# patrickltobing/shallow-wavenet

Hardware: AMD Instinct MI355X
Metric: decoded samples/sec (22.05 kHz Laplacian AR decode, whole job) (higher is better)
Workload: dtype f32

## Files before the change

### shallow_wavenet_amd/csrc/swn_decode_bl6_common.hpp

```cpp
#pragma once
#include <hip/hip_runtime.h>
#include "swn_decode_internal.hpp"

namespace swn_bl6 {

constexpr int NT = 512;
constexpr int H = 64;
constexpr int L = 6;
constexpr int RF = 64;
#ifdef SWN_STAMP
constexpr bool HEADS_ON = false;
#else
constexpr bool HEADS_ON = true;
#endif

struct Bl6Args {
    const float* P;
    SwnLayout y;
    const float* cond;
    const float* noise;
    const void* forced;
    void* out;
    float* heads;
    int B, Tf, n_steps, U, N;
    SwnNoise nz;
    const void* seed;
    int step0, resume;
    float* sess;
};

struct Bl6PoolArgs {
    Bl6Args c;
    SwnPoolTable t;
};
static_assert(sizeof(Bl6PoolArgs) <= 4096, "kernel arguments are limited to 4 KB");
struct Bl6PoolModelsArgs : Bl6PoolArgs {
    SwnPoolModels m;
};
static_assert(sizeof(Bl6PoolModelsArgs) <= 4096, "kernel arguments are limited to 4 KB");
struct Bl6W16Args : Bl6Args {
    const void* w16;
};
struct Bl6PoolW16Args : Bl6PoolArgs {
    const void* w16;
};
static_assert(sizeof(Bl6PoolW16Args) <= 4096, "kernel arguments are limited to 4 KB");
struct Bl6W16Layout {
    size_t wsk, w1, w2, total;
};
inline __host__ __device__ Bl6W16Layout w16_layout(int S, int O1, int NO, bool softmax) {
    Bl6W16Layout y;
    y.wsk = 0;
    y.w1 = y.wsk + (size_t)L * S * 64 * 2;
    y.w2 = y.w1 + (size_t)O1 * S * 2;
    y.total = y.w2 + (softmax ? (size_t)NO * O1 * 2 : 0);
    return y;
}

constexpr int cmax(int a, int b) { return a > b ? a : b; }
constexpr int pow2ceil(int x) { int r = 1; while (r < x) r <<= 1; return r; }
constexpr int r4(int x) { return (x + 3) & ~3; }

__device__ __forceinline__ __amdgpu_buffer_rsrc_t make_rsrc(const void* p, unsigned bytes) {
    return __builtin_amdgcn_make_buffer_rsrc(const_cast<void*>(p), 0, bytes, 0x00020000);
}
__device__ __forceinline__ float4 buf_ld4(__amdgpu_buffer_rsrc_t r, unsigned voff_bytes, unsigned soff_bytes) {
    return __builtin_bit_cast(float4, __builtin_amdgcn_raw_buffer_load_b128(r, voff_bytes, soff_bytes, 0));
}
__device__ __forceinline__ uint4 buf_ld4u(__amdgpu_buffer_rsrc_t r, unsigned voff_bytes, unsigned soff_bytes) {
    return __builtin_bit_cast(uint4, __builtin_amdgcn_raw_buffer_load_b128(r, voff_bytes, soff_bytes, 0));
}
__device__ __forceinline__ float w16_lo(unsigned w) { return __builtin_bit_cast(float, w << 16); }
__device__ __forceinline__ float w16_hi(unsigned w) { return __builtin_bit_cast(float, w & 0xffff0000u); }

template <int CTRL>
__device__ __forceinline__ float dpp_f(float v) {
    return __builtin_bit_cast(float, __builtin_amdgcn_update_dpp(0, __builtin_bit_cast(int, v), CTRL, 0xf, 0xf, true));
}
__device__ __forceinline__ float sum4(float v) {
    v += dpp_f<0xB1>(v);
    v += dpp_f<0x4E>(v);
    return v;
}
__device__ __forceinline__ float sum8(float v) {
    v = sum4(v);
    v += dpp_f<0x141>(v);
    return v;
}
__device__ __forceinline__ float exp_c(float x) {
    const float t = x * 1.44269504f;
    const float lo = fmaf(x, 1.44269504f, -t) + x * 1.92596299e-8f;
    const float e = __builtin_amdgcn_exp2f(t);
    return fmaf(e, lo * 0.693147181f, e);
}
__device__ __forceinline__ float rcp_c(float x) {
    const float r = __builtin_amdgcn_rcpf(x);
    return fmaf(r, fmaf(-x, r, 1.f), r);
}
__device__ __forceinline__ float sigm(float x) { return rcp_c(1.f + exp_c(-x)); }
__device__ __forceinline__ float tanh_c(float x) {
    if (fabsf(x) > 9.02f) return copysignf(1.f, x);
    const float t = exp_c(-2.f * fabsf(x));
    return copysignf((1.f - t) * rcp_c(1.f + t), x);
}
__device__ __forceinline__ float ssign(float x) { return x * rcp_c(1.f + fabsf(x)); }

__device__ __forceinline__ void lds_barrier() {
#ifdef SWN_SYNC
    __syncthreads(); return;
#endif
    __builtin_amdgcn_fence(__ATOMIC_RELEASE, "workgroup", "local");
    __builtin_amdgcn_s_barrier();
    __builtin_amdgcn_fence(__ATOMIC_ACQUIRE, "workgroup", "local");
}

#define c_b  lds[T::o_cz + o]
#define c_v0 lds[T::o_cz + H + o]
#define c_v1 lds[T::o_cz + 2 * H + o]
#define c_c0 lds[T::o_cz + 3 * H + o]
#define c_c1 lds[T::o_cz + 4 * H + o]

inline void fill_args(Bl6Args& a, const SwnDecodeCall& c) {
    swn_make_layout(&c.g, &a.y);
    a.P = c.packed; a.cond = c.cond; a.noise = c.nz.ptr; a.nz = c.nz; a.forced = c.forced; a.seed = c.seed; a.out = c.out;
    a.heads = c.heads; a.B = c.batch; a.Tf = c.n_frames; a.n_steps = c.n_steps; a.U = c.g.U; a.N = c.g.N;
    a.step0 = c.step0; a.resume = c.resume; a.sess = c.stream ? c.state : nullptr;
}

inline bool wants_ext(const Bl6Args& a) { return !a.nz.ptr || a.nz.dump || a.seed; }

template <class A>
int launch_kernel(void (*kern)(A), size_t lds_bytes, int n_groups, const A& a, hipStream_t st, const char* where) {
    if (lds_bytes > 64 * 1024 &&
        hipFuncSetAttribute(reinterpret_cast<const void*>(kern), hipFuncAttributeMaxDynamicSharedMemorySize, (int)lds_bytes) != hipSuccess)
        return SWN_E_LAUNCH;
    hipLaunchKernelGGL(kern, dim3(n_groups), dim3(NT), lds_bytes, st, a);
    return swn_launch_status(where);
}

}
```

### shallow_wavenet_amd/csrc/swn_decode_bl6w.hip

```cpp
#include <type_traits>
#include "swn_decode_bl6_common.hpp"
#include "swn_decode_internal.hpp"

namespace {

using namespace swn_bl6;

constexpr int NG = 256;
constexpr int S = 128;
constexpr int O1 = 128;

template <int LPC_, bool EXT_>
struct Tw {
    static constexpr int LPC = LPC_;
    static constexpr bool EXT = EXT_;
    using Ext = Tw<LPC_, true>;
    static constexpr int NO = 2 + LPC_;
    static constexpr int WN = cmax(1, LPC_) + 1;
    static constexpr int ring_len(int l) { return pow2ceil((1 << l) + 1); }
    static constexpr int ring_off(int l) { int o = 0; for (int i = 0; i < l; ++i) o += ring_len(i) * H; return o; }
    static constexpr int PF = L * 2 * H;
    static constexpr int NZC = 64, NZB = 4;
    static constexpr int o_ring = 0;
    static constexpr int o_hcat = o_ring + ring_off(L);
    static constexpr int o_gp = o_hcat + L * H;
    static constexpr int o_bx = o_gp + 2 * PF;
    static constexpr int o_bd = o_bx + L * 2 * H;
    static constexpr int o_old = o_bd + L * 2 * H;
    static constexpr int o_wup = o_old + 2 * L * 2 * H;
    static constexpr int o_skip = o_wup + 256;
    static constexpr int o_p2 = o_skip + S;
    static constexpr int o_tnz = o_p2 + 4 * NO;
    static constexpr int o_cz = o_tnz + r4(NZB * NZC);
    static constexpr int o_w2 = o_cz + 5 * H;
    static constexpr int o_bias = o_w2 + NO * S + r4(NO);
    static constexpr int o_w1 = o_bias + S + O1;
    static constexpr int o_wl = o_w1 + 8 * O1 * 16;
    static constexpr int o_h0w = o_wl + 8 * NG * 4;
    static constexpr int o_end = o_h0w + 3 * H;
    static constexpr size_t lds_bytes = (size_t)o_end * sizeof(float);
    static constexpr int sess_old = ring_off(L);
    static constexpr int sess_win = sess_old + 2 * L * 2 * H;
    static constexpr int sess_floats = sess_win + r4(WN);
};

__device__ __forceinline__ float sum_quads(float v) {
    v += dpp_f<0x124>(v);
    v += dpp_f<0x128>(v);
    float w = v;
    asm("s_nop 1\n\tv_permlane16_swap_b32 %0, %1" : "+v"(v), "+v"(w));
    v += w;
    w = v;
    asm("s_nop 1\n\tv_permlane32_swap_b32 %0, %1" : "+v"(v), "+v"(w));
    return v + w;
}
template <class T, int LAYER>
__device__ __forceinline__ void layer_a(float* lds, const float (&w)[2][16], const int q, const float wj, const int pb, const int ta,
                                        const float* xr) {
    const int o = ta >> 2, p = ta & 3, pr = p & 1;
    const float e_old = lds[T::o_old + (q & 1) * (L * 2 * H) + LAYER * 2 * H + pr * H + o];
    const float e_gx = fmaf(wj, lds[T::o_gp + pb + LAYER * 2 * H + pr * H + o], lds[T::o_bx + LAYER * 2 * H + pr * H + o]);
    const float e_hp = xr[o];
    float az = 0.f, ac = 0.f;
#pragma unroll
    for (int m = 0; m < 4; ++m) {
        const float4 x = *reinterpret_cast<const float4*>(xr + 16 * p + 4 * m);
        az = fmaf(w[0][4 * m], x.x, az); ac = fmaf(w[1][4 * m], x.x, ac);
        az = fmaf(w[0][4 * m + 1], x.y, az); ac = fmaf(w[1][4 * m + 1], x.y, ac);
        az = fmaf(w[0][4 * m + 2], x.z, az); ac = fmaf(w[1][4 * m + 2], x.z, ac);
        az = fmaf(w[0][4 * m + 3], x.w, az); ac = fmaf(w[1][4 * m + 3], x.w, ac);
    }
    az = sum4(az); ac = sum4(ac);
    __builtin_amdgcn_sched_barrier(0);
    if (p < 2) {
        const float sa = (p == 0 ? az : ac) + e_old;
        const float v = e_gx * sa;
        float res;
        if (fabsf(v) > 9.02f && p == 1) {
            res = copysignf(1.f, v);
        } else {
            const float e = exp_c(p == 0 ? -v : -2.f * fabsf(v));
            const float r = rcp_c(1.f + e);
            res = p == 0 ? r : copysignf((1.f - e) * r, v);
        }
        const float c = dpp_f<0xF5>(res);
        if (p == 0) {
            const float hn = (1.f - res) * c + res * e_hp;
            if (LAYER + 1 < L) {
                constexpr int R2 = T::ring_len(LAYER + 1 < L ? LAYER + 1 : LAYER);
                lds[T::o_ring + T::ring_off(LAYER + 1 < L ? LAYER + 1 : LAYER) + (q & (R2 - 1)) * H + o] = hn;
            }
            lds[T::o_hcat + LAYER * H + o] = hn;
        }
    }
    __builtin_amdgcn_sched_barrier(0);
}

template <class T, int LAYER, int MB = 4>
__device__ __forceinline__ void older_sum(const float* lds, const float (&w)[2][16], const int qn, const int tb, float& az, float& ac) {
    constexpr int dil = 1 << LAYER;
    constexpr int R = T::ring_len(LAYER);
    const int p = tb & 3;
    const float* ring = lds + T::o_ring + T::ring_off(LAYER);
    az = 0.f; ac = 0.f;
#pragma unroll
    for (int m = 0; m < 4; ++m) {
        const float4 x = *reinterpret_cast<const float4*>(ring + ((qn - dil) & (R - 1)) * H + 16 * p + 4 * m);
        float4 w0, w1;
        if (LAYER < L - 1) {
            w0 = make_float4(w[0][4 * m], w[0][4 * m + 1], w[0][4 * m + 2], w[0][4 * m + 3]);
            w1 = make_float4(w[1][4 * m], w[1][4 * m + 1], w[1][4 * m + 2], w[1][4 * m + 3]);
        } else {
            w0 = *reinterpret_cast<const float4*>(lds + T::o_wl + (m * NG + tb) * 4);
            w1 = *reinterpret_cast<const float4*>(lds + T::o_wl + ((4 + m) * NG + tb) * 4);
        }
        az = fmaf(w0.x, x.x, az); ac = fmaf(w1.x, x.x, ac);
        az = fmaf(w0.y, x.y, az); ac = fmaf(w1.y, x.y, ac);
        az = fmaf(w0.z, x.z, az); ac = fmaf(w1.z, x.z, ac);
        az = fmaf(w0.w, x.w, az); ac = fmaf(w1.w, x.w, ac);
        if (MB < 4 && m % MB == MB - 1) __builtin_amdgcn_sched_barrier(0);
    }
    az = sum4(az); ac = sum4(ac);
}
template <class T, int LAYER>
__device__ __forceinline__ void older_store(float* lds, const int qn, const int tb, const float az, const float ac) {
    const int o = tb >> 2, p = tb & 3, pr = p & 1;
    lds[T::o_old + (qn & 1) * (L * 2 * H) + LAYER * 2 * H + pr * H + o] = (p == 0 ? az : ac) + lds[T::o_bd + LAYER * 2 * H + pr * H + o];
}
template <class T, int LAYER, int MB = 4>
__device__ __forceinline__ void older_b(float* lds, const float (&w)[2][16], const int qn, const int tb) {
    float az, ac;
    older_sum<T, LAYER, MB>(lds, w, qn, tb, az, ac);
    if ((tb & 3) < 2) older_store<T, LAYER>(lds, qn, tb, az, ac);
}
template <int... LS> struct Layers {};
template <class T, int NW, int... LS>
__device__ __forceinline__ void older_bn(Layers<LS...>, float* lds, const float (&w)[NW][2][16], const int qn, const int tb) {
    static_assert(((LS < NW) && ...), "register-resident halves only");
    float az[sizeof...(LS)], ac[sizeof...(LS)];
    int k = 0;
    ((older_sum<T, LS>(lds, w[LS], qn, tb, az[k], ac[k]), ++k), ...);
    if ((tb & 3) < 2) {
        k = 0;
        ((older_store<T, LS>(lds, qn, tb, az[k], ac[k]), ++k), ...);
    }
}

template <int LAYER>
__device__ __forceinline__ void skip_issue_b(__amdgpu_buffer_rsrc_t wsk2, float4 (&wsl)[8], const int tb, const unsigned step0) {
    const int r = tb >> 2, hp = tb & 3;
#pragma unroll
    for (int ps = 0; ps < 2; ++ps)
#pragma unroll
        for (int mm = 0; mm < 4; ++mm)
            wsl[ps * 4 + mm] = buf_ld4(wsk2, (unsigned)((r + 64 * ps) * 4 + hp) * 16u, (unsigned)((LAYER * 4 + mm) * S) * 64u + step0);
}
template <class T, int LAYER>
__device__ __forceinline__ void skip_roll_b(const float* lds, __amdgpu_buffer_rsrc_t wsk2, float4 (&wsl)[8], float (&sacc)[2], const int tb,
                                            const unsigned step0) {
    static_assert(LAYER >= 1 && LAYER < L, "slice LAYER - 1 in flight, slice LAYER to request");
    const int r = tb >> 2, hp = tb & 3;
#pragma unroll
    for (int hf = 0; hf < 2; ++hf) {
#pragma unroll
        for (int mm = 2 * hf; mm < 2 * hf + 2; ++mm) {
            const float4 x = *reinterpret_cast<const float4*>(lds + T::o_hcat + (LAYER - 1) * H + 16 * mm + 4 * hp);
#pragma unroll
            for (int ps = 0; ps < 2; ++ps) {
                const float4 w = wsl[ps * 4 + mm];
                sacc[ps] = fmaf(w.x, x.x, sacc[ps]); sacc[ps] = fmaf(w.y, x.y, sacc[ps]);
                sacc[ps] = fmaf(w.z, x.z, sacc[ps]); sacc[ps] = fmaf(w.w, x.w, sacc[ps]);
            }
        }
        __builtin_amdgcn_sched_barrier(0);
#pragma unroll
        for (int mm = 2 * hf; mm < 2 * hf + 2; ++mm)
#pragma unroll
            for (int ps = 0; ps < 2; ++ps)
                wsl[ps * 4 + mm] = buf_ld4(wsk2, (unsigned)((r + 64 * ps) * 4 + hp) * 16u, (unsigned)((LAYER * 4 + mm) * S) * 64u + step0);
        __builtin_amdgcn_sched_barrier(0);
    }
    asm volatile("" : "+v"(sacc[0]), "+v"(sacc[1]));
}
template <class T>
__device__ __forceinline__ void skip_last_b(float* lds, const float4 (&wsl)[8], const float (&sacc)[2], const int tb) {
    const int r = tb >> 2, hp = tb & 3;
    float part[2][4];
#pragma unroll
    for (int mm = 0; mm < 4; ++mm) {
        const float4 x = *reinterpret_cast<const float4*>(lds + T::o_hcat + (L - 1) * H + 16 * mm + 4 * hp);
#pragma unroll
        for (int ps = 0; ps < 2; ++ps) {
            const float4 w = wsl[ps * 4 + mm];
            part[ps][mm] = fmaf(w.w, x.w, fmaf(w.z, x.z, fmaf(w.y, x.y, w.x * x.x)));
        }
    }
    float s[2];
#pragma unroll
    for (int ps = 0; ps < 2; ++ps) s[ps] = sacc[ps] + ((part[ps][0] + part[ps][1]) + (part[ps][2] + part[ps][3]));
    const float t0 = s[0] + dpp_f<0xB1>(s[0]), t1 = s[1] + dpp_f<0xB1>(s[1]);
    const float v = (hp < 2 ? t0 : t1) + dpp_f<0x4E>(hp < 2 ? t1 : t0);
    if ((hp & 1) == 0) lds[T::o_skip + r + 32 * hp] = fmaxf(v, 0.f);
}

using OlderMerged = Layers<3, 4>;
using OlderOut1 = Layers<0, 1, 2>;

template <class T, bool GA, bool STREAM, bool POOL = false>
__device__ __forceinline__ void decode_body(const Bl6Args& a, float* lds) {
    constexpr bool EXT = T::EXT;
    static_assert(!STREAM || EXT, "streamed chunks run the extended mode");
    constexpr bool grpA = GA;
    const int tid = threadIdx.x, b = POOL ? 0 : blockIdx.x;
    __builtin_assume(GA ? tid < NG : tid >= NG);
    const int tg = tid & (NG - 1);
    const float* __restrict__ P = a.P;
    const int U = a.U;
    const int s0 = STREAM ? a.step0 : 0;
    const bool resume = STREAM && a.resume;
    const int fb0 = STREAM ? s0 / U : 0;

    for (int e = tid; e < T::o_end; e += NT) lds[e] = 0.f;
    __syncthreads();
    for (int e = tid; e < L * 2 * H; e += NT) {
        lds[T::o_bx + e] = P[a.y.bx + e];
        const float bd = P[a.y.bd + e];
        lds[T::o_bd + e] = bd;
        lds[T::o_old + e] = bd;
    }
    for (int e = tid; e < U; e += NT) lds[T::o_wup + e] = P[a.y.wup + e];
    for (int e = tid; e < H; e += NT) lds[T::o_cz + e] = P[a.y.cb + e];
    for (int e = tid; e < S; e += NT) lds[T::o_bias + e] = P[a.y.bsk + e];
    for (int e = tid; e < O1; e += NT) lds[T::o_bias + S + e] = P[a.y.b1 + e];
    for (int e = tid; e < 2 * H; e += NT) { lds[T::o_cz + H + e] = P[a.y.cv + e]; lds[T::o_cz + 3 * H + e] = P[a.y.cc + e]; }
    for (int e = tid; e < T::NO * S; e += NT) lds[T::o_w2 + e] = P[a.y.w2 + (size_t)(e / S) * r4(S) + (e % S)];
    for (int e = tid; e < T::NO; e += NT) lds[T::o_w2 + T::NO * S + e] = P[a.y.b2 + e];
    for (int e = tid; e < 8 * O1 * 16; e += NT) lds[T::o_w1 + e] = P[a.y.w12 + e];
    const __amdgpu_buffer_rsrc_t condr =
        make_rsrc(a.cond + (size_t)b * a.Tf * a.N, (unsigned)((size_t)a.Tf * a.N * sizeof(float)));
    auto load_frame = [&](int fr) {
        float* dst = lds + T::o_gp + (fr & 1) * T::PF;
#pragma unroll
        for (int it = 0; it < (T::PF / 4 + NT - 1) / NT; ++it) {
            const int e4 = it * NT + tid;
            if (e4 < T::PF / 4)
                *reinterpret_cast<float4*>(dst + 4 * e4) =
                    buf_ld4(condr, (unsigned)tid * 16u, (unsigned)(fr * a.N * 4 + it * NT * 16));
        }
    };
    for (int fr = fb0; fr < fb0 + 2 && fr < a.Tf; ++fr) load_frame(fr);
    constexpr int NWR = grpA ? L : L - 1;
    float wreg[NWR][2][16];
    {
        const int o = tg >> 2, p = tg & 3, k = grpA ? 1 : 0;
#pragma unroll
        for (int l = 0; l < L; ++l)
#pragma unroll
            for (int r = 0; r < 2; ++r) {
                const float4* src = reinterpret_cast<const float4*>(P + a.y.wd + (((size_t)l * 2 * H + o + r * H) * 2 + k) * H + 16 * p);
#pragma unroll
                for (int v = 0; v < 4; ++v) {
                    const float4 t = src[v];
                    if (l == L - 1 && !grpA) {
                        *reinterpret_cast<float4*>(lds + T::o_wl + ((r * 4 + v) * NG + tg) * 4) = t;
                    } else {
                        float (&wr)[16] = wreg[l < NWR ? l : 0][r];
                        wr[4 * v] = t.x; wr[4 * v + 1] = t.y; wr[4 * v + 2] = t.z; wr[4 * v + 3] = t.w;
                    }
                }
            }
    }
    __syncthreads();
    const float* sess_b = STREAM ? a.sess + (size_t)b * T::sess_floats : nullptr;
    int tcp = tid;
    asm volatile("" : "+v"(tcp));
    if (resume) {
        for (int e = tcp; e < T::ring_off(L); e += NT) lds[T::o_ring + e] = sess_b[e];
        for (int e = tcp; e < 2 * L * 2 * H; e += NT) lds[T::o_old + e] = sess_b[T::sess_old + e];
        __syncthreads();
    }

    int fb = fb0, tb0 = fb0 * U;
    const int n_pro = RF;
    auto cond_taps = [&](int q, float& wj, int& pb) {
        const int t0 = q - RF;
        const int tlo = t0 < 0 ? 0 : t0;
        if (tlo >= tb0 + U) {
            fb += 1; tb0 += U;
            if (fb + 1 < a.Tf) load_frame(fb + 1);
        }
        int rel = tlo - tb0;
        int fsel = fb;
        if (rel >= U) { rel -= U; fsel = fb + 1; }
        rel = rel < U ? rel : U - 1;
        wj = lds[T::o_wup + rel];
        pb = (fsel & 1) * T::PF;
    };

    auto input_seed = [&](int q) {
        if (tid < H) {
            const int o = tid;
            float acc = c_b;
#pragma unroll
            for (int k = 0; k < 2; ++k) {
                const int r = q - (1 - k);
                if (r >= 0) acc += fmaf(k ? c_v1 : c_v0, 0.f, k ? c_c1 : c_c0);
            }
            lds[T::o_ring + (q & 1) * H + o] = ssign(acc);
        }
    };
    float win[T::WN];
#pragma unroll
    for (int k = 0; k < T::WN; ++k) win[k] = 0.f;
    if (EXT && a.seed) win[T::WN - 1] = reinterpret_cast<const float*>(a.seed)[b];
    if (resume) {
#pragma unroll
        for (int k = 0; k < T::WN; ++k) win[k] = sess_b[T::sess_win + k];
    }
    const int wv = __builtin_amdgcn_readfirstlane(tg >> 6);
    float kcb = 0.f, kv0 = 0.f, kv1 = 0.f, kc0 = 0.f, kc1 = 0.f;
    if (grpA) { const int o = tg & (H - 1); kcb = c_b; kv0 = c_v0; kv1 = c_v1; kc0 = c_c0; kc1 = c_c1; }
    auto h0_row = [&](int qn) -> float* {
        return wv == 0 ? lds + T::o_ring + (qn & 1) * H : lds + T::o_h0w + (wv - 1) * H;
    };
    auto input_gen = [&](int qn) {
        if constexpr (grpA) {
            float acc = kcb;
            acc += fmaf(kv0, win[T::WN - 2], kc0);
            acc += fmaf(kv1, win[T::WN - 1], kc1);
            h0_row(qn)[tg & (H - 1)] = ssign(acc);
            asm volatile("s_waitcnt lgkmcnt(0)" ::: "memory");
        }
    };
    float e_next = 0.f;
    auto noise_load = [&](int c) {
        const int step = c * T::NZC + tid - 64;
        if (step < a.n_steps) e_next = a.noise[(size_t)b * a.n_steps + step];
    };
    auto noise_chunk = [&](int c) {
        if (grpA && tid >= 64 && tid < 128) {
            const int k = tid - 64, step = c * T::NZC + k;
            if (step < a.n_steps) {
                const float e = EXT ? swn_noise_laplace_at(a.nz, b, step, s0 + step, 0, a.n_steps, 1) : e_next;
                const float sg = (e > 0.f) ? 1.f : ((e < 0.f) ? -1.f : 0.f);
                lds[T::o_tnz + (c & (T::NZB - 1)) * T::NZC + k] = sg * log1pf(-2.f * fabsf(e));
            }
            if (!EXT) noise_load(c + 1);
        }
    };
    if (!EXT && grpA && tid >= 64 && tid < 128) noise_load(0);
    noise_chunk(0);
    noise_chunk(1);

    const __amdgpu_buffer_rsrc_t wsk2 = make_rsrc(P + a.y.wsk2, (unsigned)(L * S * 64 * sizeof(float)));

#ifdef SWN_STAMP
    unsigned long long tw[9] = {0, 0, 0, 0, 0, 0, 0, 0, 0}, tv[6] = {0, 0, 0, 0, 0, 0}, tstep = 0, tlast = 0, tbeg = 0;
#define SWN_BAR(k) { tw[k] += __builtin_amdgcn_s_memtime() - tlast; lds_barrier(); tlast = __builtin_amdgcn_s_memtime(); }
#define SWN_WAIT_STAMP(k) { asm volatile("" :: "v"(wsl[0].x)); tv[k] += __builtin_amdgcn_s_memtime() - tlast; }
#else
#define SWN_BAR(k) lds_barrier();
#define SWN_WAIT_STAMP(k)
#endif
#define SWN_PHASE(LAYER, GEN, X0)                                                                                     \
    if constexpr (grpA) layer_a<T, LAYER>(lds, wreg[LAYER], q, wj, pb, tg,                                             \
                                          LAYER == 0 ? (X0) : lds + T::o_ring + T::ring_off(LAYER) +                   \
                                                                  (q & (T::ring_len(LAYER) - 1)) * H);                 \
    else {                                                                                                             \
        if (GEN) {    \
                      \
                      \
            if (LAYER == 0) skip_issue_b<0>(wsk2, wsl, tg, step0);                                                     \
            else { SWN_WAIT_STAMP(LAYER > 0 ? LAYER - 1 : 0) skip_roll_b<T, (LAYER > 0 ? LAYER : 1)>(lds, wsk2, wsl, sacc, tg, step0); } \
            __builtin_amdgcn_sched_barrier(0);                                                                         \
        }                                                                                                              \
        if (!(GEN)) older_b<T, LAYER>(lds, wreg[LAYER < NWR ? LAYER : 0], q + 1, tg);                                  \
        else if (LAYER == 0) older_bn<T>(OlderMerged{}, lds, wreg, q + 1, tg);                                         \
        __builtin_amdgcn_sched_barrier(0);                                                                             \
    }                                                                                                                  \
    if (GEN) { SWN_BAR(LAYER) } else lds_barrier();

#pragma unroll 1
    for (int q = resume ? n_pro : 0; q < n_pro; ++q) {
        float wj; int pb;
        float4 wsl[8]; float sacc[2]; const unsigned step0 = 0;
        cond_taps(q, wj, pb);
        input_seed(q);
        lds_barrier();
        const float* x0 = lds + T::o_ring + (q & 1) * H;
        SWN_PHASE(0, false, x0) SWN_PHASE(1, false, x0) SWN_PHASE(2, false, x0) SWN_PHASE(3, false, x0)
        SWN_PHASE(4, false, x0) SWN_PHASE(5, false, x0)
        (void)wsl; (void)sacc; (void)step0;
    }

    input_gen(RF + s0);
#ifdef SWN_STAMP
    tlast = tbeg = __builtin_amdgcn_s_memtime();
#endif
    auto gen_step = [&](const int i) __attribute__((always_inline)) {
        const int q = RF + s0 + i;
        float wj; int pb;
        cond_taps(q, wj, pb);
        float4 wsl[8];
        float sacc[2] = {0.f, 0.f};
        if constexpr (!grpA) {
            const float bs0 = lds[T::o_bias + (tg >> 2)], bs1 = lds[T::o_bias + (tg >> 2) + 64];
            if ((tg & 3) == 0) { sacc[0] = bs0; sacc[1] = bs1; }
        }
        unsigned step0 = 0;
        asm volatile("" : "+s"(step0));
        const float* x0 = h0_row(q);
        SWN_PHASE(0, true, x0) SWN_PHASE(1, true, x0) SWN_PHASE(2, true, x0) SWN_PHASE(3, true, x0)
        SWN_PHASE(4, true, x0) SWN_PHASE(5, true, x0)
        if constexpr (!grpA) { SWN_WAIT_STAMP(5) skip_last_b<T>(lds, wsl, sacc, tg); }
        else older_b<T, L - 1, 2>(lds, wreg[L - 1], q + 1, tg + (int)step0);
        SWN_BAR(6)
        if constexpr (grpA) {
            const int hr = tg >> 2, hp = tg & 3;
            float a0 = 0.f, a1 = 0.f, b0 = 0.f, b1 = 0.f;
#pragma unroll
            for (int mm = 0; mm < 8; ++mm) {
                const float4 x0 = *reinterpret_cast<const float4*>(lds + T::o_skip + 16 * mm + 4 * hp);
                const float4 w0 = *reinterpret_cast<const float4*>(lds + T::o_w1 + ((mm * O1 + hr) * 4 + hp) * 4);
                const float4 w1 = *reinterpret_cast<const float4*>(lds + T::o_w1 + ((mm * O1 + hr + 64) * 4 + hp) * 4);
                float& acc = (mm & 1) ? a1 : a0;
                float& bcc = (mm & 1) ? b1 : b0;
                acc = fmaf(w0.x, x0.x, acc); acc = fmaf(w0.y, x0.y, acc); acc = fmaf(w0.z, x0.z, acc); acc = fmaf(w0.w, x0.w, acc);
                bcc = fmaf(w1.x, x0.x, bcc); bcc = fmaf(w1.y, x0.y, bcc); bcc = fmaf(w1.z, x0.z, bcc); bcc = fmaf(w1.w, x0.w, bcc);
                if ((mm & 3) == 3) __builtin_amdgcn_sched_barrier(0);
            }
            const float v = sum4(a0 + a1), u = sum4(b0 + b1);
            const float o1a = fmaxf(v + lds[T::o_bias + S + hr], 0.f), o1b = fmaxf(u + lds[T::o_bias + S + hr + 64], 0.f);
#pragma unroll
            for (int j = 0; j < (T::NO + 3) / 4; ++j) {
                const int k = hp + 4 * j, kc = k < T::NO ? k : T::NO - 1;
                const float* w2 = lds + T::o_w2 + kc * S;
                const float b2 = lds[T::o_w2 + T::NO * S + kc];
                const float pz = sum_quads(fmaf(w2[hr + 64], o1b, fmaf(w2[hr], o1a, tg < 4 ? b2 : 0.f)));
                if ((tg & 63) < 4 && k < T::NO) lds[T::o_p2 + 4 * k + wv] = pz;
            }
        } else {
            older_bn<T>(OlderOut1{}, lds, wreg, q + 1, tg);
        }
        SWN_BAR(7)
        if constexpr (grpA) {
            const int ln = tg & 63;
            float tz = 0.f;
            if constexpr (!EXT) tz = lds[T::o_tnz + (i & (T::NZB * T::NZC - 1))];
            float fv = 0.f;
            if (a.forced) fv = reinterpret_cast<const float*>(a.forced)[(size_t)b * a.n_steps + i];
            const float4 pz = *reinterpret_cast<const float4*>(lds + T::o_p2 + 4 * (ln < T::NO ? ln : T::NO - 1));
            const float acc = (pz.x + pz.y) + (pz.z + pz.w);
            float o2[T::NO];
#pragma unroll
            for (int k = 0; k < T::NO; ++k) o2[k] = __builtin_bit_cast(float, __builtin_amdgcn_readlane(__builtin_bit_cast(int, acc), k));
            {
#pragma clang fp contract(off)
                float* outp = reinterpret_cast<float*>(a.out) + (size_t)b * a.n_steps + (size_t)i;
                const float mu = o2[0];
                const float bsc = sigm(o2[1]);
                float lpv = 0.f;
#pragma unroll
                for (int k = 0; k < T::LPC; ++k) lpv += o2[2 + T::LPC - 1 - k] * win[T::WN - T::LPC + k];
                const float t = bsc * (EXT ? lds[T::o_tnz + ((i >> 6) & (T::NZB - 1)) * T::NZC + (i & (T::NZC - 1))] : tz);
                float sv = (T::LPC > 0) ? (lpv + mu) - t : mu - t;
                sv = fminf(fmaxf(sv, -1.f), 1.f);
                float fd = a.forced ? fv : sv;
                asm volatile("" : "+v"(fd));
#pragma unroll
                for (int k = 0; k + 1 < T::WN; ++k) win[k] = win[k + 1];
                win[T::WN - 1] = fd;
                if (tid == 0) outp[0] = sv;
            }
            if (HEADS_ON && a.heads && wv == 0 && ln < T::NO) a.heads[((size_t)b * a.n_steps + i) * T::NO + ln] = acc;
        }
        if (i + 1 < a.n_steps) input_gen(q + 1);
#ifdef SWN_STAMP
        if constexpr (grpA) tw[8] += __builtin_amdgcn_s_memtime() - tlast;
#endif
    };
#pragma unroll 1
    for (int i0 = 0; i0 < a.n_steps; i0 += T::NZC) {
        noise_chunk((i0 >> 6) + 2);
        const int iend = i0 + T::NZC < a.n_steps ? i0 + T::NZC : a.n_steps;
#pragma unroll 1
        for (int i = i0; i < iend; ++i) gen_step(i);
    }
#ifdef SWN_STAMP
    { const unsigned long long tn = __builtin_amdgcn_s_memtime(); tw[0] += tn - tlast; tstep = tn - tbeg; }
#endif
    if constexpr (STREAM) {
        __syncthreads();
        float* so = a.sess + (size_t)b * T::sess_floats;
        tcp = tid;
        asm volatile("" : "+v"(tcp));
        for (int e = tcp; e < T::ring_off(L); e += NT) so[e] = lds[T::o_ring + e];
        for (int e = tcp; e < 2 * L * 2 * H; e += NT) so[T::sess_old + e] = lds[T::o_old + e];
        if (tid == 0) {
#pragma unroll
            for (int k = 0; k < T::WN; ++k) so[T::sess_win + k] = win[k];
        }
    }
#undef SWN_PHASE
#undef SWN_BAR
#undef SWN_WAIT_STAMP
#ifdef SWN_STAMP
    if ((tid == 0 || tid == 64 || tid == NG) && b == 0 && a.heads) {
        float* h = a.heads + (tid == 0 ? 0 : tid == 64 ? 30 : 10);
        for (int k = 0; k < 9; ++k) h[k] = (float)((double)tw[k] / (double)a.n_steps);
        if (tid == 0) h[9] = (float)((double)tstep / (double)a.n_steps);
        else if (tid == NG) for (int k = 0; k < 6; ++k) h[10 + k] = (float)((double)tv[k] / (double)a.n_steps);
    }
#endif
}

template <class T, bool STREAM = false>
__global__ __launch_bounds__(NT) void decode_bl6w_kernel(const Bl6Args a) {
    extern __shared__ __attribute__((aligned(16))) float lds[];
    if (threadIdx.x < NG) decode_body<T, true, STREAM>(a, lds);
    else decode_body<T, false, STREAM>(a, lds);
}

template <class T, bool MODELS = false>
__global__ __launch_bounds__(NT) void decode_bl6w_pool_kernel(
    const typename std::conditional<MODELS, Bl6PoolModelsArgs, Bl6PoolArgs>::type p) {
    extern __shared__ __attribute__((aligned(16))) float lds[];
    static_assert(T::EXT, "pools run the extended mode");
    Bl6Args a = p.c;
    if constexpr (MODELS) a.P = swn_pool_model(p.m);
    if (!swn_pool_entry_args(a, p.t, 1, 1, T::NO)) return;
    a.sess += (size_t)swn_pool_slot(p.t) * T::sess_floats;
    if (threadIdx.x < NG) decode_body<T, true, true, true>(a, lds);
    else decode_body<T, false, true, true>(a, lds);
}

bool bl6w_applies(const SwnGeom& g) {
    return g.bl6 && g.U <= 256 && g.U >= 2 && !g.audio_in && g.kind == SWN_KIND_LAPLACE && g.S == 128 && g.O1 == 128 &&
           g.seg == 1 && (g.lpc == 0 || g.lpc == 4);
}

template <class F>
int with_tw(const SwnGeom& g, F&& f) {
    if (!bl6w_applies(g)) return SWN_E_UNSUPPORTED;
    if (g.lpc == 0) return f(Tw<0, false>{});
    return f(Tw<4, false>{});
}

}

int swn_decode_bl6w_run(const SwnDecodeCall& c) {
    const hipStream_t st = c.hip_stream;
    if (c.pool) {
        Bl6PoolModelsArgs p;
        fill_args(p.c, c);
        p.t = *c.pool;
        if (c.models) p.m = *c.models;
        return with_tw(c.g, [&](auto tw) {
            using T = typename decltype(tw)::Ext;
            if (c.models)
                return launch_kernel(decode_bl6w_pool_kernel<T, true>, T::lds_bytes, c.batch, p, st, "swn_decode_pool_chunk_models(bl6w)");
            const Bl6PoolArgs& p1 = p;
            return launch_kernel(decode_bl6w_pool_kernel<T>, T::lds_bytes, c.batch, p1, st, "swn_decode_pool_chunk(bl6w)");
        });
    }
    Bl6Args a;
    fill_args(a, c);
    return with_tw(c.g, [&](auto t) {
        using T = decltype(t);
        using X = typename T::Ext;
        static_assert(T::lds_bytes <= 160 * 1024 && X::lds_bytes <= 160 * 1024, "LDS budget");
        if (c.stream) return launch_kernel(decode_bl6w_kernel<X, true>, X::lds_bytes, a.B, a, st, "swn_decode(bl6w)");
        if (wants_ext(a)) return launch_kernel(decode_bl6w_kernel<X>, X::lds_bytes, a.B, a, st, "swn_decode(bl6w)");
        return launch_kernel(decode_bl6w_kernel<T>, T::lds_bytes, a.B, a, st, "swn_decode(bl6w)");
    });
}

size_t swn_decode_bl6w_session_floats(const SwnGeom& g) {
    int n = 0;
    with_tw(g, [&](auto t) { n = decltype(t)::sess_floats; return SWN_OK; });
    return (size_t)n;
}
```

Measured before the change: 362,100.

## Prefetch LDS operands across barrier 6 with partial lgkmcnt wait

Adds a barrier variant that waits only until a given number of LDS loads remain outstanding, so loads issued just before the barrier can stay in flight across it. Group B issues the ring-row loads for the older-layer sums before barrier 6, and group A (when LPC==0) preloads the first W1 tiles. It also software-pipelines the W1 skip-projection loop with rotating register buffers. The aim is to hide LDS latency behind barrier wait, at the cost of more registers and relying on the loaded data not being written by other waves across that barrier.

```diff
diff --git a/shallow_wavenet_amd/csrc/swn_decode_bl6_common.hpp b/shallow_wavenet_amd/csrc/swn_decode_bl6_common.hpp
--- a/shallow_wavenet_amd/csrc/swn_decode_bl6_common.hpp
+++ b/shallow_wavenet_amd/csrc/swn_decode_bl6_common.hpp
@@ -114,6 +114,20 @@
     __builtin_amdgcn_fence(__ATOMIC_ACQUIRE, "workgroup", "local");
 }
 
+__device__ __forceinline__ void lds_fence_compiler() { asm volatile("" ::: "memory"); }
+template <int N>
+__device__ __forceinline__ void lds_barrier_keep() {
+    static_assert(N >= 0 && N <= 15, "lgkmcnt is a four-bit counter");
+#ifdef SWN_SYNC
+    __syncthreads(); return;
+#endif
+    __builtin_amdgcn_sched_barrier(0);
+    asm volatile("s_waitcnt lgkmcnt(%0)" :: "n"(N) : "memory");
+    __builtin_amdgcn_s_barrier();
+    lds_fence_compiler();
+    __builtin_amdgcn_sched_barrier(0);
+}
+
 #define c_b  lds[T::o_cz + o]
 #define c_v0 lds[T::o_cz + H + o]
 #define c_v1 lds[T::o_cz + 2 * H + o]
diff --git a/shallow_wavenet_amd/csrc/swn_decode_bl6w.hip b/shallow_wavenet_amd/csrc/swn_decode_bl6w.hip
--- a/shallow_wavenet_amd/csrc/swn_decode_bl6w.hip
+++ b/shallow_wavenet_amd/csrc/swn_decode_bl6w.hip
@@ -146,6 +146,43 @@
     }
 }
 
+template <class T, int LAYER>
+__device__ __forceinline__ void older_rows(const float* lds, const int qn, const int tb, float4 (&x)[4]) {
+    constexpr int dil = 1 << LAYER;
+    constexpr int R = T::ring_len(LAYER);
+    const float* row = lds + T::o_ring + T::ring_off(LAYER) + ((qn - dil) & (R - 1)) * H + 16 * (tb & 3);
+#pragma unroll
+    for (int m = 0; m < 4; ++m) x[m] = *reinterpret_cast<const float4*>(row + 4 * m);
+}
+__device__ __forceinline__ void older_sum_x(const float (&w)[2][16], const float4 (&x)[4], float& az, float& ac) {
+    az = 0.f; ac = 0.f;
+#pragma unroll
+    for (int m = 0; m < 4; ++m) {
+        az = fmaf(w[0][4 * m], x[m].x, az); ac = fmaf(w[1][4 * m], x[m].x, ac);
+        az = fmaf(w[0][4 * m + 1], x[m].y, az); ac = fmaf(w[1][4 * m + 1], x[m].y, ac);
+        az = fmaf(w[0][4 * m + 2], x[m].z, az); ac = fmaf(w[1][4 * m + 2], x[m].z, ac);
+        az = fmaf(w[0][4 * m + 3], x[m].w, az); ac = fmaf(w[1][4 * m + 3], x[m].w, ac);
+    }
+    az = sum4(az); ac = sum4(ac);
+}
+template <class T, int... LS>
+__device__ __forceinline__ void older_rows_n(Layers<LS...>, const float* lds, const int qn, const int tb, float4 (&x)[sizeof...(LS)][4]) {
+    int k = 0;
+    ((older_rows<T, LS>(lds, qn, tb, x[k]), ++k), ...);
+}
+template <class T, int NW, int... LS>
+__device__ __forceinline__ void older_bn_x(Layers<LS...>, float* lds, const float (&w)[NW][2][16], const float4 (&x)[sizeof...(LS)][4],
+                                           const int qn, const int tb) {
+    static_assert(((LS < NW) && ...), "register-resident halves only");
+    float az[sizeof...(LS)], ac[sizeof...(LS)];
+    int k = 0;
+    ((older_sum_x(w[LS], x[k], az[k], ac[k]), ++k), ...);
+    if ((tb & 3) < 2) {
+        k = 0;
+        ((older_store<T, LS>(lds, qn, tb, az[k], ac[k]), ++k), ...);
+    }
+}
+
 template <int LAYER>
 __device__ __forceinline__ void skip_issue_b(__amdgpu_buffer_rsrc_t wsk2, float4 (&wsl)[8], const int tb, const unsigned step0) {
     const int r = tb >> 2, hp = tb & 3;
@@ -358,9 +395,13 @@
     unsigned long long tw[9] = {0, 0, 0, 0, 0, 0, 0, 0, 0}, tv[6] = {0, 0, 0, 0, 0, 0}, tstep = 0, tlast = 0, tbeg = 0;
 #define SWN_BAR(k) { tw[k] += __builtin_amdgcn_s_memtime() - tlast; lds_barrier(); tlast = __builtin_amdgcn_s_memtime(); }
 #define SWN_WAIT_STAMP(k) { asm volatile("" :: "v"(wsl[0].x)); tv[k] += __builtin_amdgcn_s_memtime() - tlast; }
+#define SWN_PRE(k) { tw[k] += __builtin_amdgcn_s_memtime() - tlast; asm volatile("s_waitcnt lgkmcnt(0)" ::: "memory"); }
+#define SWN_BAR_KEEP(k, N) { lds_barrier_keep<N>(); tlast = __builtin_amdgcn_s_memtime(); }
 #else
 #define SWN_BAR(k) lds_barrier();
 #define SWN_WAIT_STAMP(k)
+#define SWN_PRE(k)
+#define SWN_BAR_KEEP(k, N) lds_barrier_keep<N>();
 #endif
 #define SWN_PHASE(LAYER, GEN, X0)                                                                                     \
     if constexpr (grpA) layer_a<T, LAYER>(lds, wreg[LAYER], q, wj, pb, tg,                                             \
@@ -412,22 +453,62 @@
         const float* x0 = h0_row(q);
         SWN_PHASE(0, true, x0) SWN_PHASE(1, true, x0) SWN_PHASE(2, true, x0) SWN_PHASE(3, true, x0)
         SWN_PHASE(4, true, x0) SWN_PHASE(5, true, x0)
-        if constexpr (!grpA) { SWN_WAIT_STAMP(5) skip_last_b<T>(lds, wsl, sacc, tg); }
-        else older_b<T, L - 1, 2>(lds, wreg[L - 1], q + 1, tg + (int)step0);
-        SWN_BAR(6)
+        constexpr bool ROLL1 = T::LPC == 0;
+        float4 xo[3][4];
+        float4 w1e[2][2];
+        if constexpr (!grpA) {
+            SWN_WAIT_STAMP(5) skip_last_b<T>(lds, wsl, sacc, tg);
+            SWN_PRE(6)
+            lds_fence_compiler();
+            __builtin_amdgcn_sched_barrier(0);
+            older_rows_n<T>(OlderOut1{}, lds, q + 1, tg, xo);
+            __builtin_amdgcn_sched_barrier(0);
+            SWN_BAR_KEEP(6, 12)
+        } else {
+            older_b<T, L - 1, 2>(lds, wreg[L - 1], q + 1, tg + (int)step0);
+            if constexpr (ROLL1) {
+                SWN_PRE(6)
+                lds_fence_compiler();
+                __builtin_amdgcn_sched_barrier(0);
+#pragma unroll
+                for (int mm = 0; mm < 2; ++mm)
+#pragma unroll
+                    for (int r = 0; r < 2; ++r)
+                        w1e[mm][r] = *reinterpret_cast<const float4*>(lds + T::o_w1 + ((mm * O1 + (tg >> 2) + 64 * r) * 4 + (tg & 3)) * 4);
+                __builtin_amdgcn_sched_barrier(0);
+                SWN_BAR_KEEP(6, 4)
+            } else {
+                SWN_BAR(6)
+            }
+        }
         if constexpr (grpA) {
             const int hr = tg >> 2, hp = tg & 3;
             float a0 = 0.f, a1 = 0.f, b0 = 0.f, b1 = 0.f;
-#pragma unroll
-            for (int mm = 0; mm < 8; ++mm) {
-                const float4 x0 = *reinterpret_cast<const float4*>(lds + T::o_skip + 16 * mm + 4 * hp);
-                const float4 w0 = *reinterpret_cast<const float4*>(lds + T::o_w1 + ((mm * O1 + hr) * 4 + hp) * 4);
-                const float4 w1 = *reinterpret_cast<const float4*>(lds + T::o_w1 + ((mm * O1 + hr + 64) * 4 + hp) * 4);
+            auto X = [&](int mm) { return *reinterpret_cast<const float4*>(lds + T::o_skip + 16 * mm + 4 * hp); };
+            auto W = [&](int mm, int r) { return *reinterpret_cast<const float4*>(lds + T::o_w1 + ((mm * O1 + hr + 64 * r) * 4 + hp) * 4); };
+            auto fma8 = [&](int mm, const float4& x0, const float4& w0, const float4& w1) {
                 float& acc = (mm & 1) ? a1 : a0;
                 float& bcc = (mm & 1) ? b1 : b0;
                 acc = fmaf(w0.x, x0.x, acc); acc = fmaf(w0.y, x0.y, acc); acc = fmaf(w0.z, x0.z, acc); acc = fmaf(w0.w, x0.w, acc);
                 bcc = fmaf(w1.x, x0.x, bcc); bcc = fmaf(w1.y, x0.y, bcc); bcc = fmaf(w1.z, x0.z, bcc); bcc = fmaf(w1.w, x0.w, bcc);
-                if ((mm & 3) == 3) __builtin_amdgcn_sched_barrier(0);
+            };
+            if constexpr (ROLL1) {
+                float4 xr[3] = {X(0), X(1), X(2)};
+                __builtin_amdgcn_sched_barrier(0);
+#pragma unroll
+                for (int mm = 0; mm < 8; ++mm) {
+                    fma8(mm, xr[mm % 3], w1e[mm % 2][0], w1e[mm % 2][1]);
+                    __builtin_amdgcn_sched_barrier(0);
+                    if (mm + 2 < 8) { w1e[mm % 2][0] = W(mm + 2, 0); w1e[mm % 2][1] = W(mm + 2, 1); }
+                    if (mm + 3 < 8) xr[mm % 3] = X(mm + 3);
+                    __builtin_amdgcn_sched_barrier(0);
+                }
+            } else {
+#pragma unroll
+                for (int mm = 0; mm < 8; ++mm) {
+                    fma8(mm, X(mm), W(mm, 0), W(mm, 1));
+                    if ((mm & 3) == 3) __builtin_amdgcn_sched_barrier(0);
+                }
             }
             const float v = sum4(a0 + a1), u = sum4(b0 + b1);
             const float o1a = fmaxf(v + lds[T::o_bias + S + hr], 0.f), o1b = fmaxf(u + lds[T::o_bias + S + hr + 64], 0.f);
@@ -440,7 +521,7 @@
                 if ((tg & 63) < 4 && k < T::NO) lds[T::o_p2 + 4 * k + wv] = pz;
             }
         } else {
-            older_bn<T>(OlderOut1{}, lds, wreg, q + 1, tg);
+            older_bn_x<T>(OlderOut1{}, lds, wreg, xo, q + 1, tg);
         }
         SWN_BAR(7)
         if constexpr (grpA) {
@@ -504,6 +585,8 @@
 #undef SWN_PHASE
 #undef SWN_BAR
 #undef SWN_WAIT_STAMP
+#undef SWN_PRE
+#undef SWN_BAR_KEEP
 #ifdef SWN_STAMP
     if ((tid == 0 || tid == 64 || tid == NG) && b == 0 && a.heads) {
         float* h = a.heads + (tid == 0 ? 0 : tid == 64 ? 30 : 10);
```

New measurement: 372,600 (median of 6 runs). 1.03x the previous value.
